# amcpherson/defuse

Hardware: AMD Instinct MI355X
Metric: split-read DP aligns/sec (higher is better)
Workload: dtype int16

## Files before the change

### defuse_amd/csrc/dsa_diag.hpp

```cpp
#pragma once
#include <hip/hip_runtime.h>

namespace dsa {

#ifdef DSA_NO_PRUNE
constexpr bool DIAG_PRUNE = false;
#else
constexpr bool DIAG_PRUNE = true;
#endif
#ifdef DSA_NO_GAP_SKIP
constexpr bool DIAG_GAP_SKIP = false;
#else
constexpr bool DIAG_GAP_SKIP = true;
#endif
#ifdef DSA_ABLATE_TAIL
constexpr bool DIAG_TAIL = false;
#else
constexpr bool DIAG_TAIL = true;
#endif
#ifdef DSA_ABLATE_REPLAY
constexpr bool DIAG_REPLAY = false;
#else
constexpr bool DIAG_REPLAY = true;
#endif

enum DiagSlot {
    DS_GROUPS_SKIPPED = 0, DS_GROUPS = 1, DS_UNUSED2 = 2, DS_WAVE_CYCLES = 3, DS_BARRIER = 4, DS_TABLES = 5, DS_TAIL = 6, DS_ROWMAX = 7,
    DS_COMBINE = 8, DS_REPLAY = 9, DS_GREPLAY_SETUP = 10, DS_GREPLAY_SWEEP = 11, DS_GREPLAY_WAVES = 12, DS_GREPLAY_STEPS = 13,
    DS_GAP_GROUPS = 14, DS_SLOWEST_LISTED = 15,
    DS_TILE_GROUPS = 16,
    DS_TILE_CYCLES = 32,
    DS_TILE_SLOTS = 16, DS_SLOTS = 48
};

#ifdef DSA_PRUNE_STATS
struct DiagClock {
    unsigned long long t;
    __device__ DiagClock() : t(__builtin_readcyclecounter()) {}
    __device__ unsigned long long lap()
    {
        const unsigned long long n = __builtin_readcyclecounter(), d = n - t;
        t = n;
        return d;
    }
};
#define DSA_STAT_ADD(g, slot, v) atomicAdd(&(g).stats[slot], (unsigned long long)(v))
#define DSA_STAT_MAX(g, slot, v) atomicMax(&(g).stats[slot], (unsigned long long)(v))
#else
struct DiagClock {
    __device__ unsigned long long lap() { return 0; }
};
#define DSA_STAT_ADD(g, slot, v) ((void)0)
#define DSA_STAT_MAX(g, slot, v) ((void)0)
#endif

}
```

### defuse_amd/csrc/dsa_kernels.hpp

```cpp
#pragma once
#include <hip/hip_runtime.h>
#include <stdint.h>

#include "../../include/defuse_dsa.h"
#include "dsa_diag.hpp"
#include "dsa_tile.hpp"

namespace dsa {

constexpr int W = TILE_W;
constexpr int WAVE = 64;
constexpr int WG_WAVES = 4;
constexpr int WG_LANES = WG_WAVES * WAVE;
constexpr uint32_t REF_PAD16 = 0x00AAu;
constexpr uint32_t ROW_PAD16 = 0x0055u;

constexpr int NCLS = 5;
constexpr int NCOMBO = NCLS * NCLS;
constexpr int TROW = W + 4;
#ifndef FILL_PF
#define FILL_PF 2
#endif
constexpr int GMAX = 4;
constexpr int TGROUP = NCOMBO * TROW;
// ... 79 lines not shown
    for (int j = 1; j < GMAX; ++j)
        if (k == j) f = v.f4[j];
    return f;
}
__device__ __forceinline__ WgView wg_groups(WgGroupsLds* gl, int f, int f_prev_of_wave_lane0, int& my_group)
{
    const int tid = threadIdx.x, lane = tid & 63, wv = tid >> 6;
    int fprev = __shfl_up(f, 1, 64);
    if (lane == 0) fprev = f_prev_of_wave_lane0;
    const bool start = tid == 0 || f != fprev;
    const unsigned long long m = __builtin_amdgcn_ballot_w64(start);
    if (lane == 0) gl->wave_starts[wv] = __builtin_popcountll(m);
    __syncthreads();
    int base = 0, total = 0;
#pragma unroll
    for (int k = 0; k < WG_WAVES; ++k) {
        const int c = gl->wave_starts[k];
        if (k < wv) base += c;
        total += c;
    }
    my_group = base + __builtin_popcountll(m & ((2ull << lane) - 1ull)) - 1;
    if (start && my_group < GSPLIT2) gl->group_f[my_group] = f;
    __syncthreads();
    total = uniform(total);
    WgView v;
    v.n_groups = total <= GSPLIT2 ? total : 0;
    v.list = gl->group_f;
#pragma unroll
    for (int k = 0; k < GMAX; ++k) v.f4[k] = k < total ? uniform(gl->group_f[k]) : 0;
    return v;
}

struct Geom {
    int32_t n_waves;
    int32_t n_wgs;
    int32_t lq1;
    int32_t nch;
    int32_t lrp;
    int32_t wt;
    int32_t n_fusions;
    int64_t n_pairs;
    const int32_t* orig;
    uint32_t tiers_launched;
#ifdef DSA_PRUNE_STATS
    unsigned long long* stats;
#endif
};

struct KeptRow {
    int16_t a;
    int16_t m1, m2;
    int16_t pad_;
};

constexpr uint8_t NO_CHUNK = 0xFF;
struct ReplayTask {
    uint32_t pair;
    uint32_t mask_begin;
    uint16_t last_row;
    uint8_t  chunk0;
    uint8_t  chunk1;
    int32_t fusion;
};
constexpr uint32_t GTASK_OWNER = 0x80000000u;
constexpr uint16_t TASK_FAST = 0x8000u;
constexpr uint16_t TASK_ONLY = 0x4000u;
constexpr uint16_t TASK_ROW = 0x3FFFu;

struct alignas(8) PairState {
    uint32_t mask_begin;
    uint32_t kept_begin;
    uint32_t task_begin;
    uint16_t n_kept;
    uint8_t n_tasks;
    uint8_t flags;
    uint16_t tiles0, tiles1;
    uint8_t first0, first1;
    uint16_t pad_;
};
__device__ __forceinline__ int task_of_tile(uint32_t tiles, int first, int c)
{
    if (c == first) return 0;
    const uint32_t rest = first < 16 ? tiles & ~(1u << first) : tiles;
    return 1 + __builtin_popcount(rest & ((1u << c) - 1u));
}
static_assert(sizeof(PairState) == 24, "three 8-byte loads");
constexpr uint8_t STATE_COUNTED = 1;
constexpr uint8_t STATE_TILES = 2;

struct Counters {
    unsigned long long n_kept, n_tasks, n_masks, n_gtasks;
    unsigned need_tiers;
    unsigned pad_;
    unsigned fill_wgs[8];
};
constexpr int FILL_WGS_FAST = 0;
constexpr int FILL_WGS_GENERIC = 6;

__device__ __forceinline__ int cdiv_dev(int a, int b) { return (a + b - 1) / b; }

__host__ __device__ __forceinline__ int64_t rowidx(int j, int lane) { return ((int64_t)(j >> 2) * WAVE + lane) * 4 + (j & 3); }
constexpr uint32_t CODE_MASK = 0xFF00FF00u;
__device__ __forceinline__ int half_of(uint32_t v, int h) { return (int)((v >> (16 * h)) & 0xFFFFu) - (int)BIAS16; }

typedef uint32_t u32x4 __attribute__((ext_vector_type(4)));
__device__ __forceinline__ uint4 load_group(const uint4* p)
{
    const u32x4 v = *reinterpret_cast<const u32x4*>(p);
    return make_uint4(v.x, v.y, v.z, v.w);
}
__device__ __forceinline__ void wait_loads() { __builtin_amdgcn_s_waitcnt(0x0F70); }

__global__ void k_pack_refs(const uint8_t* __restrict__ ref_bytes, const dsa_fusion* __restrict__ fusions,
                            uint32_t* __restrict__ refcodes, Geom g)
{
    int64_t t = (int64_t)blockIdx.x * blockDim.x + threadIdx.x;
    int64_t total = (int64_t)g.n_fusions * g.lrp;
    if (t >= total) return;
    const int s = (int)(t % g.lrp), k = s % W;
    const int i = (s / W) * g.wt + k;
    const dsa_fusion f = fusions[t / g.lrp];
    uint32_t lo = REF_PAD16, hi = REF_PAD16;
    if (k >= g.wt) {
        refcodes[t] = lo | (hi << 16);
        return;
    }
    if (i < f.ref0_len) lo = (uint32_t)ref_bytes[(int64_t)f.ref0_off + i] << 8;
    if (i < f.ref1_len) hi = (uint32_t)ref_bytes[(int64_t)f.ref1_off + (f.ref1_len - 1 - i)] << 8;
    refcodes[t] = lo | (hi << 16);
}

__device__ __forceinline__ bool is_fast_base(uint32_t b)
{
    return b == 'A' || b == 'C' || b == 'G' || b == 'T' || b == 'N';
}

__device__ __forceinline__ uint32_t base_class(uint32_t byte)
{
    uint32_t k = (byte >> 1) & 7u;
    return k > 4u ? 4u : k;
}
__device__ __forceinline__ uint32_t table_row(uint32_t k1, uint32_t k2)
{
    if (k1 < 4u && k2 < 4u) return 4u * k1 + k2;
    return k1 == 4u ? 16u + k2 : 21u + k1;
}
__device__ __forceinline__ void table_row_classes(int t, int& k1, int& k2)
{
    if (t < 16) { k1 = t >> 2; k2 = t & 3; }
    else if (t < 21) { k1 = 4; k2 = t - 16; }
    else { k1 = t - 21; k2 = 4; }
}

template <bool SPLIT, int WT, class CodeFn>
__device__ __forceinline__ void build_tables(uint32_t* __restrict__ T, int n_groups, CodeFn&& code_of)
{
    for (int e = threadIdx.x; e < n_groups * WT; e += WG_LANES) {
        const int i = e % WT, gi = e / WT;
        uint32_t q0, q1;
        code_of(gi, i, q0, q1);
        const uint32_t cls_byte[NCLS] = {'A', 'C', 'T', 'G', 'N'};
        uint32_t lo[NCLS], hi[NCLS];
#pragma unroll
        for (int k = 0; k < NCLS; ++k) {
            lo[k] = q0 == REF_PAD16 ? 0u : ((q0 >> 8) == cls_byte[k] ? 4u : 1u);
            hi[k] = (q1 == REF_PAD16 ? 0u : ((q1 >> 8) == cls_byte[k] ? 4u : 1u)) << 16;
        }
        const uint32_t drift = i > 0 ? TWO2 : 0u;
        if (SPLIT) {
            unsigned short* col = reinterpret_cast<unsigned short*>(T + gi * TGROUP_SPLIT) + i;
#pragma unroll
            for (int k = 0; k < NCLS; ++k) {
                col[k * TROW] = (unsigned short)(lo[k] + (drift & 0xFFFFu));
                col[(NCLS + k) * TROW] = (unsigned short)((hi[k] + (drift & 0xFFFF0000u)) >> 16);
            }
        } else {
            uint32_t* col = T + gi * TGROUP + i;
#pragma unroll
            for (int t = 0; t < NCOMBO; ++t) {
                int k1, k2;
                table_row_classes(t, k1, k2);
                col[t * TROW] = (lo[k1] | hi[k2]) + drift;
            }
        }
    }
}

template <int BYTE_KIND>
__device__ __forceinline__ bool pack_rows_wave(const uint8_t* __restrict__ read_bytes, const dsa_pair* __restrict__ pairs,
                                               uint32_t* __restrict__ rowcodes, uint32_t* __restrict__ row_bytes, const Geom& g, int w,
                                               int lane, int lq_wave)
{
    const int64_t p = (int64_t)w * WAVE + lane;
    const bool valid = p < g.n_pairs;
    dsa_pair pr{};
    if (valid) pr = pairs[p];
    uint4* out = reinterpret_cast<uint4*>(rowcodes + (int64_t)w * g.lq1 * WAVE) + lane;
    uint32_t* out1 = BYTE_KIND ? row_bytes + (int64_t)w * (g.lq1 >> 2) * WAVE + lane : nullptr;
    bool exotic = false;
    for (int gq = 0; gq <= (lq_wave >> 2); ++gq) {
        uint32_t code[4];
        uint32_t bytes = 0;
#pragma unroll
        for (int sidx = 0; sidx < 4; ++sidx) {
            const int j = 4 * gq + sidx;
            code[sidx] = ROW_PAD16 | (ROW_PAD16 << 16);
            if (valid && j >= 1 && j <= pr.read_len) {
                const uint32_t b0 = read_bytes[(int64_t)pr.read_off + (j - 1)];
                const uint32_t b1 = read_bytes[(int64_t)pr.read_off + (pr.read_len - j)];
                exotic |= !is_fast_base(b0);
                const uint32_t k1 = base_class(b0), k2 = base_class(b1);
                code[sidx] = (b0 << 8) | (b1 << 24) | table_row(k1, k2) | ((k1 | (k2 << 4)) << 16);
                if (BYTE_KIND) bytes |= (BYTE_KIND == 1 ? table_row(k1, k2) : (k1 | (k2 << 4))) << (8 * sidx);
            }
        }
        out[(int64_t)gq * WAVE] = make_uint4(code[0], code[1], code[2], code[3]);
        if (BYTE_KIND) out1[(int64_t)gq * WAVE] = bytes;
    }
    return exotic;
}

template <int WT>
__device__ __forceinline__ void row_step(uint32_t (&X)[WT], const uint32_t (&r)[WT], uint32_t cj, uint32_t bprev,
                                         uint32_t bcur)
{
    cj &= CODE_MASK;
    constexpr int BLK = 16;
    uint32_t a = (bprev + FOUR2) - min3u(cj ^ r[0]);
    uint32_t up = bcur - TWO2;
#pragma unroll
    for (int b = 0; b < WT; b += BLK) {
        uint32_t d[BLK];
#pragma unroll
        for (int k = 0; k < BLK; ++k)
            d[k] = b + k + 1 < WT ? SIX2 - min3u(cj ^ r[b + k + 1]) : 0u;
#pragma unroll
        for (int k = 0; k < BLK && b + k < WT; ++k) {
            const int i = b + k;
            const uint32_t a_next = X[i] + d[k];
            X[i] = max3(a, X[i], up);
            up = X[i];
            a = a_next;
        }
    }
}

template <bool MASKED, int WT>
__device__ __forceinline__ uint32_t tile_row_max(const uint32_t (&X)[WT], int nv0, int nv1)
{
    uint32_t acc0 = BIAS2, acc1 = BIAS2;
    static_assert(WT % 4 == 0, "four columns per step");
#pragma unroll
    for (int i = 0; i < WT; i += 4) {
        uint32_t x[4];
#pragma unroll
        for (int k = 0; k < 4; ++k) {
            x[k] = X[i + k] - drift2(i + k);
            if (MASKED) {
                if (i + k >= nv0) x[k] = (x[k] & 0xFFFF0000u) | BIAS16;
                if (i + k >= nv1) x[k] = (x[k] & 0x0000FFFFu) | (BIAS16 << 16);
            }
        }
        acc0 = max3(acc0, x[0], x[1]);
        acc1 = max3(acc1, x[2], x[3]);
    }
    return max2(acc0, acc1);
}

__device__ __forceinline__ unsigned long long wave_alloc(unsigned long long* counter, unsigned n)
{
    unsigned incl = n;
#pragma unroll
    for (int d = 1; d < 64; d <<= 1) {
        unsigned y = __shfl_up(incl, d, 64);
        if ((int)(threadIdx.x & 63) >= d) incl += y;
    }
    const unsigned total = __shfl(incl, 63, 64);
    unsigned long long base = 0;
    if ((threadIdx.x & 63) == 63 && total) base = atomicAdd(counter, (unsigned long long)total);
    base = __shfl(base, 63, 64);
    return base + (incl - n);
}

__device__ __forceinline__ int nth_set_bit(uint64_t m, int n)
{
    for (int k = 0; k < n && m; ++k) m &= m - 1;
    return m ? __builtin_ctzll(m) : -1;
}

struct TileStops { int v[8]; };

struct FinishBufs {
    PairState* state;
    KeptRow* kept;
    ReplayTask* tasks;
    uint64_t* masks;
    uint2* gtasks;
    Counters* ctr;
    uint64_t kept_cap, task_cap, mask_cap, gtask_cap;
    int32_t* tstop;
    int64_t* rec_count;
};

struct EmitOut {
    const int64_t* rec_offset;
    dsa_record* out;
    uint64_t out_cap;
    int64_t pair_base;
};

__device__ __forceinline__ bool finish_void(const FinishBufs& fb, const Geom& g)
{
    const Counters* __restrict__ ctr = fb.ctr;
    return ctr->n_tasks > fb.task_cap || ctr->n_masks > fb.mask_cap || ctr->n_kept > fb.kept_cap || ctr->n_gtasks > fb.gtask_cap ||
           (ctr->need_tiers & ~g.tiers_launched) != 0;
}

__device__ __forceinline__ uint64_t mask_half(const uint4& v, int h) { return h ? ((uint64_t)v.w << 32) | v.z : ((uint64_t)v.y << 32) | v.x; }

__device__ __forceinline__ int load_tstop(const int32_t* p) { return __hip_atomic_load(p, __ATOMIC_RELAXED, __HIP_MEMORY_SCOPE_AGENT); }

struct LaneInfo {
    uint32_t kept_begin, mask_begin;
    uint16_t n_kept;
    uint16_t last_row;
    uint8_t  c0, c1;
    uint16_t key_group;
    uint16_t lq;
    uint8_t  nv0, nv1;
};
constexpr int KCACHE = 3;
struct FinishLds {
    int tile[GSPLIT2];
    int hist[258];
    unsigned short order[WG_LANES];
    LaneInfo info[WG_LANES];
    uint64_t kc[KCACHE * WG_LANES];
};
// ... 785 lines not shown
        if (gn < stop_prev) b_n = load_group(bi4 + (int64_t)gn * WAVE);
        const uint32_t bv[4] = {b.x, b.y, b.z, b.w};
        uint32_t cmv[4] = {BIAS2, BIAS2, BIAS2, BIAS2}, bov[4] = {BIAS2, BIAS2, BIAS2, BIAS2};
        uint32_t alive_bits = 0;
#pragma unroll
        for (int sidx = 0; sidx < 4; ++sidx) {
            const int j = 4 * gq + sidx;
            const uint32_t bcur = bv[sidx];
            if (j >= 1 && j <= lq_max) {
                if constexpr (SPLIT) {
                    const uint32_t k1 = (rc >> (8 * sidx)) & 0xFu, k2 = (rc >> (8 * sidx + 4)) & 0xFu;
                    uint4 v = split_terms(tb, k1, k2, 0);
                    uint32_t a = bprev + v.x;
                    uint32_t up = bcur - TWO2;
#pragma unroll
                    for (int q = 0; q < NW / 4; ++q) {
                        uint4 vn = v;
                        if (q + 1 < NW / 4) vn = split_terms(tb, k1, k2, q + 1);
                        uint32_t an;
                        an = X[4 * q + 0] + v.y;
                        X[4 * q + 0] = max3(a, X[4 * q + 0], up);
                        a = an;
                        an = X[4 * q + 1] + v.z;
                        X[4 * q + 1] = max3(a, X[4 * q + 1], X[4 * q + 0]);
                        a = an;
                        an = X[4 * q + 2] + v.w;
                        X[4 * q + 2] = max3(a, X[4 * q + 2], X[4 * q + 1]);
                        a = an;
                        an = X[4 * q + 3] + vn.x;
                        X[4 * q + 3] = max3(a, X[4 * q + 3], X[4 * q + 2]);
                        a = an;
                        up = X[4 * q + 3];
                        v = vn;
                    }
                } else {
                    const uint4* trow = reinterpret_cast<const uint4*>(tb + ((rc >> (8 * sidx)) & 0xFFu) * TROW);
                    uint4 vq[FILL_PF + 1];
#pragma unroll
                    for (int k = 0; k <= FILL_PF; ++k) vq[k] = trow[k];
                    uint32_t a = bprev + vq[0].x;
                    uint32_t up = bcur - TWO2;
#pragma unroll
                    for (int q = 0; q < NW / 4; ++q) {
                        const uint4 v = vq[0];
#pragma unroll
                        for (int k = 0; k < FILL_PF; ++k) vq[k] = vq[k + 1];
                        if (q + 1 + FILL_PF < NW / 4) vq[FILL_PF] = trow[q + 1 + FILL_PF];
                        const uint4 vn = vq[0];
                        uint32_t an;
                        an = X[4 * q + 0] + v.y;
                        X[4 * q + 0] = max3(a, X[4 * q + 0], up);
                        a = an;
                        an = X[4 * q + 1] + v.z;
                        X[4 * q + 1] = max3(a, X[4 * q + 1], X[4 * q + 0]);
                        a = an;
                        an = X[4 * q + 2] + v.w;
                        X[4 * q + 2] = max3(a, X[4 * q + 2], X[4 * q + 1]);
                        a = an;
                        an = X[4 * q + 3] + vn.x;
                        X[4 * q + 3] = max3(a, X[4 * q + 3], X[4 * q + 2]);
                        a = an;
                        up = X[4 * q + 3];
                    }
                }
                {
                    uint32_t acc0 = BIAS2, acc1 = BIAS2;
#pragma unroll
                    for (int i = 0; i < NW; i += 4) {
                        acc0 = max3(acc0, X[i] - drift2(i), X[i + 1] - drift2(i + 1));
                        acc1 = max3(acc1, X[i + 2] - drift2(i + 2), X[i + 3] - drift2(i + 3));
                    }
                    cmv[sidx] = max2(acc0, acc1);
                }
                const uint32_t tm2 = thr_of_row(thr0, j, j <= lq_lane);
                alive_bits |= pk_max_u16(cmv[sidx], tm2) ^ tm2;
                if (!LAST) {
                    bov[sidx] = X[NW - 1] - drift2(NW - 1);
                    if ((pk_max_u16(bov[sidx], tm2) ^ tm2) != 0u) last_bnd = j;
                }
            }
            bprev = bcur;
        }
        const bool alive = alive_bits != 0u;
        cm4[(int64_t)gq * WAVE] = make_uint4(cmv[0], cmv[1], cmv[2], cmv[3]);
        if (!LAST) bo4[(int64_t)gq * WAVE] = make_uint4(bov[0], bov[1], bov[2], bov[3]);
        if (DIAG_PRUNE && __builtin_amdgcn_ballot_w64(alive) == 0) {
            if (4 * gq + 3 > l_in) { ++gq; break; }
            if (DIAG_GAP_SKIP) {
                int g2 = gq + 1;
                bool resume = false;
                uint4 bb = b_n;
                uint32_t in_prev = bv[3];
                for (; g2 < ngq; ++g2) {
                    if (g2 > gq + 1) {
                        bb = bias4;
                        if (g2 < stop_prev) bb = load_group(bi4 + (int64_t)g2 * WAVE);
                    }
                    const uint32_t bbv[5] = {in_prev, bb.x, bb.y, bb.z, bb.w};
                    uint32_t in_bits = 0;
#pragma unroll
                    for (int sidx = 0; sidx < 5; ++sidx) {
                        const int j = 4 * g2 + sidx - 1;
                        const uint32_t tm2 = thr_of_row(thr0, j, j <= lq_lane);
                        in_bits |= pk_max_u16(bbv[sidx], tm2) ^ tm2;
                    }
                    if (__builtin_amdgcn_ballot_w64(in_bits != 0u) != 0) { resume = true; break; }
                    cm4[(int64_t)g2 * WAVE] = bias4;
                    if (!LAST) bo4[(int64_t)g2 * WAVE] = bias4;
                    in_prev = bb.w;
                    if (4 * g2 + 3 > l_in) { ++g2; break; }
                }
                n_gap_groups += g2 - (gq + 1);
                if (!resume) { gq = g2; break; }
#pragma unroll
                for (int i = 0; i < NW; ++i) X[i] = BIAS2 + drift2(i);
                bprev = in_prev;
                b_n = bb;
                rc_n = rows1[(int64_t)g2 * WAVE];
                wait_loads();
                gq = g2 - 1;
            }
        }
    }
    if ((threadIdx.x & 63) == 0) {
        DSA_STAT_ADD(g, DS_GAP_GROUPS, n_gap_groups);
        DSA_STAT_ADD(g, DS_GROUPS_SKIPPED, ngq - gq);
        DSA_STAT_ADD(g, DS_GROUPS, ngq);
        DSA_STAT_ADD(g, DS_TILE_GROUPS + (tile < DS_TILE_SLOTS ? tile : DS_TILE_SLOTS - 1), gq - n_gap_groups);
    }
    return gq;
}

__host__ __device__ constexpr int tier_of(int n_groups) { return n_groups <= GMAX ? 0 : n_groups <= GSPLIT ? 1 : 2; }
#ifndef DSA_FAST_WGS
#define DSA_FAST_WGS 4
#endif
template <int TIER, bool WIDE, int WT>
__global__ __launch_bounds__(WG_LANES, TIER == 2 ? 2 : DSA_FAST_WGS) void k_fill_fast(const dsa_pair* __restrict__ pairs,
                                                           uint8_t* __restrict__ wg_tier,
                                                           const uint32_t* __restrict__ refcodes,
                                                           const uint8_t* __restrict__ read_bytes,
                                                           uint32_t* __restrict__ rowcodes, uint32_t* __restrict__ row_bytes,
                                                           const int32_t* __restrict__ min_score_tab,
                                                           const dsa_fusion* __restrict__ fusions,
                                                           uint32_t* __restrict__ bnd, uint32_t* __restrict__ cmax,
                                                           uint32_t* __restrict__ rmax,
                                                           FinishBufs fb, Geom g)
{
    constexpr bool SPLIT = TIER > 0;
    __shared__ __attribute__((aligned(16))) uint32_t T[TIER == 2 ? GSPLIT2 * TGROUP_SPLIT : GMAX * TGROUP];
    __shared__ int s_nch, s_exotic;
    __shared__ FinishLds fl;
    __shared__ WgGroupsLds gl;
    if (TIER != 0 && wg_tier[blockIdx.x] != TIER) return;
    const int w = __builtin_amdgcn_readfirstlane((int)(blockIdx.x * WG_WAVES + (threadIdx.x >> 6)));
    const bool live = w < g.n_waves;
    const int lane = threadIdx.x & 63;
    const int64_t p = (int64_t)w * WAVE + lane;
    const bool in_batch = p < g.n_pairs;
    const dsa_pair pr = pairs[min(p, g.n_pairs - 1)];
    const int f = pr.fusion_idx;
    int my_group;
    const WgView wgi = wg_groups(&gl, f, (lane == 0 && threadIdx.x != 0) ? pairs[min(p - 1, g.n_pairs - 1)].fusion_idx : -1, my_group);
    if (TIER == 0) {
        const int tier = wgi.n_groups == 0 ? (int)TIER_GENERIC : tier_of(wgi.n_groups);
        if (threadIdx.x == 0) {
            wg_tier[blockIdx.x] = (uint8_t)tier;
            if (tier != 0) atomicOr(&fb.ctr->need_tiers, 1u << tier);
        }
        if (tier != 0) return;
    }
    int lq_lane = 0, slack = 0, tiles_lane = 0;
    if (in_batch) {
        const dsa_fusion fu = fusions[f];
        lq_lane = pr.read_len;
        slack = 2 * lq_lane - max(min_score_tab[lq_lane], pair_bound(pr));
        tiles_lane = max(cdiv_dev(fu.ref0_len, WT), cdiv_dev(fu.ref1_len, WT));
    }
    auto wave_max = [](int v) {
#pragma unroll
        for (int d = 32; d >= 1; d >>= 1) v = max(v, __shfl_xor(v, d, 64));
        return uniform(v);
    };
    WaveInfo wi;
    wi.lq_max = wave_max(lq_lane);
    wi.nch_max = wave_max(tiles_lane);
    int l_in = wave_max(lq_lane > 0 ? min(slack >> 2, lq_lane) : 0);
    const bool exotic = live && pack_rows_wave<SPLIT ? 2 : 1>(read_bytes, pairs, rowcodes, row_bytes, g, w, lane, wi.lq_max);
    if (threadIdx.x == 0) { s_nch = 0; s_exotic = 0; }
    __syncthreads();
    if (lane == 0 && live) atomicMax(&s_nch, wi.nch_max);
    if (__builtin_amdgcn_ballot_w64(exotic) != 0 && lane == 0) atomicOr(&s_exotic, 1);
    __syncthreads();
    if (uniform(s_exotic) != 0) {
        if (threadIdx.x == 0) {
            wg_tier[blockIdx.x] = TIER_GENERIC;
            atomicOr(&fb.ctr->need_tiers, 1u << TIER_GENERIC);
        }
        return;
    }
    if (threadIdx.x == 0) atomicAdd(&fb.ctr->fill_wgs[FILL_WGS_FAST + 2 * TIER + (WIDE ? 1 : 0)], 1u);
    const int nch_wg = uniform(s_nch);

    const uint32_t* tb = T + my_group * (SPLIT ? TGROUP_SPLIT : TGROUP);
    const uint32_t* rows1 = row_bytes + (int64_t)w * (g.lq1 >> 2) * WAVE + lane;
    const uint32_t thr0 = thr_base(slack);
    int stop_prev = 0;
    TileStops stops = {};

    DiagClock clk_all, clk;
    unsigned long long t_bar = 0, t_tab = 0;
    for (int c = 0; c < nch_wg; ++c) {
        clk.lap();
        __syncthreads();
        t_bar += clk.lap();
        build_tables<SPLIT, WT>(T, wgi.n_groups, [&](int gi, int i, uint32_t& q0, uint32_t& q1) {
            const uint32_t code = refcodes[(int64_t)group_fusion(wgi, gi) * g.lrp + c * W + i];
            q0 = code & 0xFFFFu;
            q1 = code >> 16;
        });
        t_tab += clk.lap();
        __syncthreads();
        t_bar += clk.lap();
        if (!live || c >= wi.nch_max) continue;

        uint4* cm4 = reinterpret_cast<uint4*>(cmax + ((int64_t)w * g.nch + c) * g.lq1 * WAVE) + lane;
        uint4* bo4 = reinterpret_cast<uint4*>(bnd + ((int64_t)w * g.nch + c) * g.lq1 * WAVE) + lane;
        const uint4* bi4 = reinterpret_cast<const uint4*>(bnd + ((int64_t)w * g.nch + (c - 1)) * g.lq1 * WAVE) + lane;
        int last_bnd = 0, gq;
        if (c + 1 < wi.nch_max)
            gq = sweep_tile_fast<WT, SPLIT, false>(tb, rows1, bi4, cm4, bo4, c == 0, wi.lq_max, lq_lane, thr0, l_in, stop_prev, last_bnd, g, c);
        else
            gq = sweep_tile_fast<WT, SPLIT, true>(tb, rows1, bi4, cm4, bo4, c == 0, wi.lq_max, lq_lane, thr0, l_in, stop_prev, last_bnd, g, c);
        if (lane == 0) DSA_STAT_ADD(g, DS_TILE_CYCLES + (c < DS_TILE_SLOTS ? c : DS_TILE_SLOTS - 1), clk.lap());
        if (lane == 0) fb.tstop[(int64_t)w * g.nch + c] = gq;
        stop_prev = gq;
#pragma unroll
        for (int k = 0; k < 8; ++k)
            if (k == c) stops.v[k] = gq;
        l_in = wave_max(last_bnd);
    }
    clk.lap();
    unsigned long long t_rowmax = 0, t_combine = 0, t_replay = 0;
    if (DIAG_TAIL) {
        if (live) {
            __builtin_amdgcn_fence(__ATOMIC_RELEASE, "workgroup");
            reduce_row_max<WIDE>(cmax, rmax, fb.tstop, stops, g, w, lane, wi.nch_max, wi.lq_max);
        }
        t_rowmax = clk.lap();
        combine_wg<true, WT>(pairs, fusions, cmax, rmax, stops, min_score_tab, wgi, my_group, true, &fl, fb, g);
        t_combine = clk.lap();
        if (DIAG_REPLAY) replay_fast_wg<SPLIT, WT>(T, &fl, wgi, fb, refcodes, rowcodes, bnd, g);
        t_replay = clk.lap();
    }
    if (lane == 0 && live) {
        DSA_STAT_ADD(g, DS_WAVE_CYCLES, clk_all.lap());
        DSA_STAT_ADD(g, DS_BARRIER, t_bar);
        DSA_STAT_ADD(g, DS_TABLES, t_tab);
        DSA_STAT_ADD(g, DS_TAIL, t_rowmax + t_combine + t_replay);
        DSA_STAT_ADD(g, DS_ROWMAX, t_rowmax);
        DSA_STAT_ADD(g, DS_COMBINE, t_combine);
        DSA_STAT_ADD(g, DS_REPLAY, t_replay);
    }
    (void)t_bar; (void)t_tab; (void)t_rowmax; (void)t_combine; (void)t_replay;
}

constexpr int REPLAY_BLOCK = 256;
constexpr int RQ = 4;
constexpr int RW = W / RQ;
constexpr int REPLAY_TASKS = REPLAY_BLOCK / RQ;

__device__ __forceinline__ void row_step_quarter(uint32_t (&X)[RW], const uint32_t (&r)[RW], uint32_t cj, uint32_t bprev, uint32_t bcur)
{
    cj &= CODE_MASK;
    uint32_t d[RW];
#pragma unroll
    for (int k = 0; k < RW; ++k) d[k] = k + 1 < RW ? SIX2 - min3u(cj ^ r[k + 1]) : 0u;
    uint32_t a = (bprev + FOUR2) - min3u(cj ^ r[0]);
    uint32_t up = bcur - TWO2;
#pragma unroll
    for (int i = 0; i < RW; ++i) {
        const uint32_t a_next = X[i] + d[i];
        X[i] = max3(a, X[i], up);
        up = X[i];
        a = a_next;
    }
}

__device__ __forceinline__ uint32_t equal_columns_quarter(const uint32_t (&X)[RW], uint32_t target2)
{
    static_assert(RW == 16, "one accumulator word");
    const uint32_t below = target2 - 0x00010001u;
    uint32_t acc = 0;
#pragma unroll
    for (int k = RW - 1; k >= 0; --k) {
        typedef unsigned short us2 __attribute__((ext_vector_type(2)));
        const uint32_t c = below + drift2(k);
        const uint32_t y = __builtin_bit_cast(uint32_t, __builtin_elementwise_sub_sat(__builtin_bit_cast(us2, X[k]), __builtin_bit_cast(us2, c)));
        asm("v_lshl_or_b32 %0, %0, 1, %1" : "+v"(acc) : "v"(y));
    }
    return acc;
}

__global__ __launch_bounds__(REPLAY_BLOCK, 5) void k_replay(FinishBufs fb, const dsa_pair* __restrict__ pairs,
                                                   const dsa_fusion* __restrict__ fusions,
                                                   const uint32_t* __restrict__ refcodes,
                                                   const uint32_t* __restrict__ rowcodes,
                                                   const uint32_t* __restrict__ bnd, Geom g)
{
    const ReplayTask* __restrict__ tasks = fb.tasks;
    const uint2* __restrict__ gtasks = fb.gtasks;
    const PairState* __restrict__ state = fb.state;
    const KeptRow* __restrict__ kept = fb.kept;
    const int32_t* __restrict__ tstop = fb.tstop;
    uint64_t* __restrict__ masks = fb.masks;
    __shared__ int s_hist[258];
    __shared__ unsigned short s_order[REPLAY_TASKS];
    __shared__ ReplayTask s_task[REPLAY_TASKS];
    __shared__ uint64_t s_kc[KCACHE * REPLAY_BLOCK];
    static_assert(REPLAY_BLOCK == WG_LANES, "kept_row() strides the cache by WG_LANES");
    const unsigned long long n_g = fb.ctr->n_gtasks;
    if (finish_void(fb, g)) return;
    const int q = threadIdx.x & (RQ - 1);
    const int slot = threadIdx.x / RQ;
    for (unsigned long long base = (unsigned long long)blockIdx.x * REPLAY_TASKS; base < n_g;
         base += (unsigned long long)gridDim.x * REPLAY_TASKS) {
        __syncthreads();
        for (int e = threadIdx.x; e < 258; e += REPLAY_BLOCK) s_hist[e] = 0;
        __syncthreads();
        int my_key = 256, my_rank = 0;
        if (threadIdx.x < REPLAY_TASKS) {
            if (base + threadIdx.x < n_g) {
                const ReplayTask mine = tasks[gtasks[base + threadIdx.x].x & ~GTASK_OWNER];
                s_task[threadIdx.x] = mine;
                my_key = min((int)(mine.last_row & TASK_ROW), 255);
            }
            my_rank = atomicAdd(&s_hist[my_key], 1);
        }
        __syncthreads();
        if (threadIdx.x == 0) {
            int run = 0;
            for (int e = 0; e < 257; ++e) {
                const int n = s_hist[e];
                s_hist[e] = run;
                run += n;
            }
        }
        __syncthreads();
        if (threadIdx.x < REPLAY_TASKS) s_order[s_hist[my_key] + my_rank] = (unsigned short)threadIdx.x;
        __syncthreads();
        const int src = s_order[slot];
        const bool valid = base + src < n_g;
        if (__builtin_amdgcn_ballot_w64(valid) == 0) continue;
        ReplayTask rt = s_task[valid ? src : s_order[0]];
        if (!valid) { rt.last_row = 0; rt.chunk0 = rt.chunk1 = NO_CHUNK; }
        DiagClock clk;
        const int64_t p = rt.pair;
        const int64_t w = p >> 6;
        const int lane = (int)(p & 63);
        const bool has0 = rt.chunk0 != NO_CHUNK, has1 = rt.chunk1 != NO_CHUNK;
        const int c0 = has0 ? rt.chunk0 : 0, c1 = has1 ? rt.chunk1 : 0;
        const uint32_t* rc = refcodes + (int64_t)rt.fusion * g.lrp;
        const dsa_fusion fu = fusions[rt.fusion];
        PairState st = state[p];
        if (!valid) st.n_kept = 0;
        const int lq = pairs[p].read_len;
        const uint32_t* rows = rowcodes + w * g.lq1 * WAVE;
        const uint32_t* bi0 = bnd + (w * g.nch + (c0 - 1)) * g.lq1 * WAVE;
        const uint32_t* bi1 = bnd + (w * g.nch + (c1 - 1)) * g.lq1 * WAVE;
        const KeptRow* kr = kept + st.kept_begin;

        uint32_t r[RW];
#pragma unroll
        for (int i = 0; i < RW; ++i) {
            const uint32_t lo = has0 ? (rc[c0 * W + q * RW + i] & 0xFFFFu) : REF_PAD16;
// ... 437 lines not shown
```

Before: 342.1 million.

## Prefetch next tile's reference codes into registers and stage them through LDS

The per-tile table build now reads reference codes from an LDS stash instead of global memory. The next tile's codes are loaded into registers before the barrier and written to the stash (aliased onto the FinishLds region) after the table build. The first tile's codes are prefetched alongside row packing. This hides global load latency on the table-build path, at the cost of extra registers per thread and reuse of the finish LDS area, which must not be live during the fill loop.

```diff
diff --git a/defuse_amd/csrc/dsa_diag.hpp b/defuse_amd/csrc/dsa_diag.hpp
--- a/defuse_amd/csrc/dsa_diag.hpp
+++ b/defuse_amd/csrc/dsa_diag.hpp
@@ -2,6 +2,12 @@
 #include <hip/hip_runtime.h>
 
 namespace dsa {
+
+#ifdef DSA_NO_STAGE_TABLES
+constexpr bool DIAG_STAGE_TABLES = false;
+#else
+constexpr bool DIAG_STAGE_TABLES = true;
+#endif
 
 #ifdef DSA_NO_PRUNE
 constexpr bool DIAG_PRUNE = false;
diff --git a/defuse_amd/csrc/dsa_kernels.hpp b/defuse_amd/csrc/dsa_kernels.hpp
--- a/defuse_amd/csrc/dsa_kernels.hpp
+++ b/defuse_amd/csrc/dsa_kernels.hpp
@@ -255,6 +255,34 @@
     else { k1 = t - 21; k2 = 4; }
 }
 
+template <bool SPLIT>
+__device__ __forceinline__ void build_table_column(uint32_t* __restrict__ T, int gi, int i, uint32_t q0, uint32_t q1)
+{
+    const uint32_t cls_byte[NCLS] = {'A', 'C', 'T', 'G', 'N'};
+    uint32_t lo[NCLS], hi[NCLS];
+#pragma unroll
+    for (int k = 0; k < NCLS; ++k) {
+        lo[k] = q0 == REF_PAD16 ? 0u : ((q0 >> 8) == cls_byte[k] ? 4u : 1u);
+        hi[k] = (q1 == REF_PAD16 ? 0u : ((q1 >> 8) == cls_byte[k] ? 4u : 1u)) << 16;
+    }
+    const uint32_t drift = i > 0 ? TWO2 : 0u;
+    if (SPLIT) {
+        unsigned short* col = reinterpret_cast<unsigned short*>(T + gi * TGROUP_SPLIT) + i;
+#pragma unroll
+        for (int k = 0; k < NCLS; ++k) {
+            col[k * TROW] = (unsigned short)(lo[k] + (drift & 0xFFFFu));
+            col[(NCLS + k) * TROW] = (unsigned short)((hi[k] + (drift & 0xFFFF0000u)) >> 16);
+        }
+    } else {
+        uint32_t* col = T + gi * TGROUP + i;
+#pragma unroll
+        for (int t = 0; t < NCOMBO; ++t) {
+            int k1, k2;
+            table_row_classes(t, k1, k2);
+            col[t * TROW] = (lo[k1] | hi[k2]) + drift;
+        }
+    }
+}
 template <bool SPLIT, int WT, class CodeFn>
 __device__ __forceinline__ void build_tables(uint32_t* __restrict__ T, int n_groups, CodeFn&& code_of)
 {
@@ -262,31 +290,33 @@
         const int i = e % WT, gi = e / WT;
         uint32_t q0, q1;
         code_of(gi, i, q0, q1);
-        const uint32_t cls_byte[NCLS] = {'A', 'C', 'T', 'G', 'N'};
-        uint32_t lo[NCLS], hi[NCLS];
-#pragma unroll
-        for (int k = 0; k < NCLS; ++k) {
-            lo[k] = q0 == REF_PAD16 ? 0u : ((q0 >> 8) == cls_byte[k] ? 4u : 1u);
-            hi[k] = (q1 == REF_PAD16 ? 0u : ((q1 >> 8) == cls_byte[k] ? 4u : 1u)) << 16;
-        }
-        const uint32_t drift = i > 0 ? TWO2 : 0u;
-        if (SPLIT) {
-            unsigned short* col = reinterpret_cast<unsigned short*>(T + gi * TGROUP_SPLIT) + i;
-#pragma unroll
-            for (int k = 0; k < NCLS; ++k) {
-                col[k * TROW] = (unsigned short)(lo[k] + (drift & 0xFFFFu));
-                col[(NCLS + k) * TROW] = (unsigned short)((hi[k] + (drift & 0xFFFF0000u)) >> 16);
-            }
-        } else {
-            uint32_t* col = T + gi * TGROUP + i;
-#pragma unroll
-            for (int t = 0; t < NCOMBO; ++t) {
-                int k1, k2;
-                table_row_classes(t, k1, k2);
-                col[t * TROW] = (lo[k1] | hi[k2]) + drift;
-            }
-        }
-    }
+        build_table_column<SPLIT>(T, gi, i, q0, q1);
+    }
+}
+__host__ __device__ constexpr int tier_groups(int tier) { return tier == 0 ? GMAX : tier == 1 ? GSPLIT : GSPLIT2; }
+__host__ __device__ constexpr int stage_slots(int tier) { return (tier_groups(tier) * W + WG_LANES - 1) / WG_LANES; }
+template <int NS>
+struct StagedCodes {
+    uint32_t v[NS];
+};
+template <int NS, int WT>
+__device__ __forceinline__ void stage_issue(StagedCodes<NS>& s, const uint32_t* __restrict__ refcodes, const int32_t* group_f, int n_groups,
+                                            int64_t lrp, int c)
+{
+    const int last = max(n_groups * WT - 1, 0);
+#pragma unroll
+    for (int k = 0; k < NS; ++k) {
+        const int e = min(k * WG_LANES + (int)threadIdx.x, last);
+        s.v[k] = refcodes[(int64_t)group_f[e / WT] * lrp + c * W + e % WT];
+    }
+}
+template <int NS>
+__device__ __forceinline__ void stage_store(uint32_t* __restrict__ stash, const StagedCodes<NS>& s, int wave_in_wg)
+{
+    int lane = (int)__builtin_amdgcn_mbcnt_hi(~0u, __builtin_amdgcn_mbcnt_lo(~0u, 0u));
+    asm volatile("" : "+v"(lane));
+#pragma unroll
+    for (int k = 0; k < NS; ++k) stash[k * WG_LANES + wave_in_wg * WAVE + lane] = s.v[k];
 }
 
 template <int BYTE_KIND>
@@ -1378,6 +1408,9 @@
     __shared__ int s_nch, s_exotic;
     __shared__ FinishLds fl;
     __shared__ WgGroupsLds gl;
+    constexpr int NS = stage_slots(TIER);
+    static_assert(NS * WG_LANES * sizeof(uint32_t) <= sizeof(FinishLds), "the stash lies on FinishLds");
+    uint32_t* const stash = reinterpret_cast<uint32_t*>(&fl);
     if (TIER != 0 && wg_tier[blockIdx.x] != TIER) return;
     const int w = __builtin_amdgcn_readfirstlane((int)(blockIdx.x * WG_WAVES + (threadIdx.x >> 6)));
     const bool live = w < g.n_waves;
@@ -1412,7 +1445,12 @@
     wi.lq_max = wave_max(lq_lane);
     wi.nch_max = wave_max(tiles_lane);
     int l_in = wave_max(lq_lane > 0 ? min(slack >> 2, lq_lane) : 0);
+    const int n_groups = uniform(wgi.n_groups);
+    const int wave_in_wg = uniform((int)(threadIdx.x >> 6));
+    StagedCodes<NS> sc = {};
+    if (DIAG_STAGE_TABLES) stage_issue<NS, WT>(sc, refcodes, gl.group_f, n_groups, g.lrp, 0);
     const bool exotic = live && pack_rows_wave<SPLIT ? 2 : 1>(read_bytes, pairs, rowcodes, row_bytes, g, w, lane, wi.lq_max);
+    if (DIAG_STAGE_TABLES) stage_store(stash, sc, wave_in_wg);
     if (threadIdx.x == 0) { s_nch = 0; s_exotic = 0; }
     __syncthreads();
     if (lane == 0 && live) atomicMax(&s_nch, wi.nch_max);
@@ -1438,15 +1476,18 @@
     unsigned long long t_bar = 0, t_tab = 0;
     for (int c = 0; c < nch_wg; ++c) {
         clk.lap();
+        const bool stage_next = DIAG_STAGE_TABLES && c + 1 < nch_wg;
+        if (stage_next) stage_issue<NS, WT>(sc, refcodes, gl.group_f, n_groups, g.lrp, c + 1);
         __syncthreads();
         t_bar += clk.lap();
-        build_tables<SPLIT, WT>(T, wgi.n_groups, [&](int gi, int i, uint32_t& q0, uint32_t& q1) {
-            const uint32_t code = refcodes[(int64_t)group_fusion(wgi, gi) * g.lrp + c * W + i];
+        build_tables<SPLIT, WT>(T, n_groups, [&](int gi, int i, uint32_t& q0, uint32_t& q1) {
+            const uint32_t code = DIAG_STAGE_TABLES ? stash[gi * WT + i] : refcodes[(int64_t)group_fusion(wgi, gi) * g.lrp + c * W + i];
             q0 = code & 0xFFFFu;
             q1 = code >> 16;
         });
         t_tab += clk.lap();
         __syncthreads();
+        if (stage_next) stage_store(stash, sc, wave_in_wg);
         t_bar += clk.lap();
         if (!live || c >= wi.nch_max) continue;
 
```

New measurement: 340.9 million. Within noise of the previous version (-0.4%).
